# GeWu-Lab/Crab

Hardware: AMD Instinct MI355X
Metric: clips/sec prefill+decode (AVQA 10s clip, 8 frames, 256 out tok) (higher is better)
Workload: dtype bf16

## Files before the change

crab_amd/csrc/skinny.hip:

```cpp
#include "common.h"
#include "crab_internal.h"
#include "fp8_common.h"
#include "gemm_epilogue.h"
#include <stdlib.h>

namespace {

struct SkinnyP {
    const bf16_t* A; const bf16_t* B; void* C; const bf16_t* bias; const bf16_t* R;
    const bf16_t* A2; const bf16_t* B2;
    long lda, ldb, ldc, ldr, lda2, ldb2;
    int M, N, K, K2, act, c_fp32;
    float res_scale;
    const bf16_t* Bx; long ldbx; float* Tx;
    const float* rope_tab; bf16_t* rope_kc; bf16_t* rope_vc; const int* rope_pos_dev;
    int rope_H, rope_Hk, rope_d, rope_Tmax, rope_pos0;
    const int* rope_row_off;
    const uint8_t* B8; long ldb8; const float* bscale;
};

constexpr int SK_WAVES = 8;
constexpr int SKX = 8;

template <int MT, int NT>
__global__ __launch_bounds__(SK_WAVES * 64) void gemm_skinny_kernel(SkinnyP p) {
    constexpr int U = (NT + MT) <= 3 ? 4 : ((NT + MT) <= 6 ? 2 : 1);
    __shared__ __attribute__((aligned(16))) float red[SK_WAVES][NT * MT][64][4];
    const int tid = threadIdx.x, lane = tid & 63, wave = tid >> 6;
    const int fr = lane & 15, fg = lane >> 4;
    const int n0 = blockIdx.x * 16 * NT;

    const int ks1 = (p.K + 31) >> 5;
    const int ks2 = p.A2 ? (p.K2 + 31) >> 5 : 0;
    const int ks = ks1 + ks2;
    const int s_begin = (int)((long)ks * wave / SK_WAVES), s_end = (int)((long)ks * (wave + 1) / SK_WAVES);
    const int nst = s_end - s_begin;
    const int rot = nst > 0 ? (int)(blockIdx.x % (unsigned)nst) : 0;

    f32x4_t acc[NT][MT];
#pragma unroll
    for (int j = 0; j < NT; ++j)
#pragma unroll
        for (int i = 0; i < MT; ++i) acc[j][i] = f32x4_t{0.f, 0.f, 0.f, 0.f};
    long woff[NT];
#pragma unroll
    for (int j = 0; j < NT; ++j) woff[j] = min(n0 + j * 16 + fr, p.N - 1);
    int mrow[MT];
#pragma unroll
    for (int i = 0; i < MT; ++i) mrow[i] = min(i * 16 + fr, p.M - 1);

    const u32x4 z4 = {0u, 0u, 0u, 0u};
    for (int s = 0; s < nst; s += U) {
        u32x4 wv[U][NT], xv[U][MT];
#pragma unroll
        for (int u = 0; u < U; ++u) {
            const bool live = s + u < nst;
            int q = s + u + rot;
            if (q >= nst) q -= nst;
            const int st = live ? s_begin + q : s_begin;
            const bool seg2 = st >= ks1;
            const bf16_t* Bp = seg2 ? p.B2 : p.B;
            const bf16_t* Ap = seg2 ? p.A2 : p.A;
            const long lb = seg2 ? p.ldb2 : p.ldb, la = seg2 ? p.lda2 : p.lda;
            const int Kseg = seg2 ? p.K2 : p.K;
            const int k = ((seg2 ? st - ks1 : st) << 5) + fg * 8;
            const bool ok = live && k < Kseg;
            const int kc = ok ? k : 0;
#pragma unroll
            for (int j = 0; j < NT; ++j) {
                u32x4 w = *reinterpret_cast<const u32x4*>(Bp + woff[j] * lb + kc);
                wv[u][j] = ok ? w : z4;
            }
#pragma unroll
            for (int i = 0; i < MT; ++i) xv[u][i] = *reinterpret_cast<const u32x4*>(Ap + (long)mrow[i] * la + kc);
        }
#pragma unroll
        for (int u = 0; u < U; ++u) {
#pragma unroll
            for (int j = 0; j < NT; ++j) {
                union { u32x4 r; bf16x8_t f; } wf;
                wf.r = wv[u][j];
#pragma unroll
                for (int i = 0; i < MT; ++i) {
                    union { u32x4 r; bf16x8_t f; } xf;
                    xf.r = xv[u][i];
                    acc[j][i] = __builtin_amdgcn_mfma_f32_16x16x32_bf16(wf.f, xf.f, acc[j][i], 0, 0, 0);
                }
            }
        }
    }
#pragma unroll
    for (int j = 0; j < NT; ++j)
#pragma unroll
        for (int i = 0; i < MT; ++i) *reinterpret_cast<f32x4_t*>(&red[wave][j * MT + i][lane][0]) = acc[j][i];
    __syncthreads();

    for (int idx = tid; idx < NT * MT * 64; idx += SK_WAVES * 64) {
        const int t = idx >> 6, l = idx & 63;
        const int j = t / MT, i = t % MT;
        const int m = i * 16 + (l & 15);
        const int n = n0 + j * 16 + (l >> 4) * 4;
        if (m >= p.M || n >= p.N) continue;
        f32x4_t v = *reinterpret_cast<const f32x4_t*>(&red[0][t][l][0]);
#pragma unroll
        for (int w = 1; w < SK_WAVES; ++w) v += *reinterpret_cast<const f32x4_t*>(&red[w][t][l][0]);
        if (p.act == ACT_SWIGLU_PAIR) gemm_epilogue_scalar_swiglu(v, m, n, p.bias, p.C, p.ldc, p.c_fp32);
        else gemm_epilogue_scalar4(v, m, n, p.N, p.bias, p.act, p.R, p.ldr, p.res_scale, p.C, p.ldc, p.c_fp32);
    }
}

__device__ __attribute__((aligned(16))) uint32_t g_zero_page_sk[64];

typedef __attribute__((address_space(3))) void* sk_lds_vptr;
typedef const __attribute__((address_space(1))) void* sk_gbl_vptr;

struct SkRole {
    bool extra;
    int xe, n0, Nw;
    bool rope, r_qk;
    int r_hh, r_j, r_base, r_half;
    long wrow[2];
    int chunk[2];
    int fofs0, fofs1;
    __device__ __forceinline__ int rope_dim(int cg) const { return r_qk ? (cg >> 1) * r_half + 8 * r_j + (cg & 1) * 4 : 16 * r_j + cg * 4; }
};

template <int CH>
__device__ __forceinline__ SkRole sk_role(const SkinnyP& p, int lane) {
    SkRole k;
    const int nbN = (p.N + 15) / 16;
    k.extra = (int)blockIdx.x >= nbN;
    k.xe = (int)blockIdx.x - nbN;
    k.Nw = k.extra ? 16 : p.N;
    k.n0 = k.extra ? 0 : (int)blockIdx.x * 16;
    k.rope = p.rope_tab != nullptr && !k.extra;
    const int r_bpd = k.rope ? p.rope_d >> 4 : 1;
    k.r_hh = (int)blockIdx.x / r_bpd; k.r_j = (int)blockIdx.x % r_bpd;
    k.r_qk = k.rope && k.r_hh < p.rope_H + p.rope_Hk;
    k.r_base = k.r_hh * p.rope_d; k.r_half = p.rope_d >> 1;
#pragma unroll
    for (int i = 0; i < 2; ++i) {
        const int row = i * 8 + (lane >> 3);
        k.chunk[i] = (lane & 7) ^ ((row >> 1) & 7);
        k.wrow[i] = min(k.n0 + row, k.Nw - 1);
        if (k.r_qk) k.wrow[i] = k.r_base + (row >> 3) * k.r_half + 8 * k.r_j + (row & 7);
    }
    const int fr = lane & 15, fg = lane >> 4;
    k.fofs0 = fr * 8 * CH + ((fg ^ ((fr >> 1) & 7)) * CH);
    k.fofs1 = k.fofs0 ^ (4 * CH);
    return k;
}

template <typename V4>
__device__ __forceinline__ void sk_rope_tail(const SkinnyP& p, const SkRole& k, int l, const V4& s) {
    const int m = l & 15, cg = l >> 4;
    const int d = p.rope_d, pos = p.rope_pos0 + (p.rope_pos_dev ? p.rope_pos_dev[0] : 0);
    const int dim = k.rope_dim(cg);
    const int col = k.r_base + dim;
    float x[4], px[4];
#pragma unroll
    for (int r = 0; r < 4; ++r) {
        x[r] = bf2f(f2bf(s[r] + (p.bias ? bf2f(p.bias[col + r]) : 0.f)));
        px[r] = __shfl_xor(x[r], 32, 64);
    }
    if (m >= p.M) return;
    bf16_t* crow = reinterpret_cast<bf16_t*>(p.C) + (long)m * p.ldc + col;
    const uint32_t raw0 = pack_bf2(x[0], x[1]), raw1 = pack_bf2(x[2], x[3]);
    if (!k.r_qk) {
        const int hk = k.r_hh - p.rope_H - p.rope_Hk;
        *reinterpret_cast<u32x2*>(crow) = u32x2{raw0, raw1};
        *reinterpret_cast<u32x2*>(p.rope_vc + (((long)m * p.rope_Hk + hk) * p.rope_Tmax + pos) * d + dim) = u32x2{raw0, raw1};
        return;
    }
    const int idim = 8 * k.r_j + (cg & 1) * 4;
    const int rp = pos - (p.rope_row_off ? p.rope_row_off[m] : 0);
    const float* cs = p.rope_tab + ((long)rp * k.r_half + idim) * 2;
    float o[4];
#pragma unroll
    for (int r = 0; r < 4; ++r) {
        const float c = cs[2 * r], sn = cs[2 * r + 1];
        o[r] = cg < 2 ? rope_lo(x[r], px[r], c, sn) : rope_hi(px[r], x[r], c, sn);
    }
    const u32x2 ow = {pack_bf2(o[0], o[1]), pack_bf2(o[2], o[3])};
    if (k.r_hh < p.rope_H) {
        *reinterpret_cast<u32x2*>(crow) = ow;
    } else {
        const int hk = k.r_hh - p.rope_H;
        *reinterpret_cast<u32x2*>(crow) = u32x2{raw0, raw1};
        *reinterpret_cast<u32x2*>(p.rope_kc + (((long)m * p.rope_Hk + hk) * p.rope_Tmax + pos) * d + dim) = ow;
    }
}

template <typename V4>
__device__ __forceinline__ void sk_store(const SkinnyP& p, float* part, const V4& v, int m, int n) {
    if (part) gemm_epilogue_scalar4(v, m, n, p.N, p.bias, p.act, p.R, p.ldr, p.res_scale, part, p.N, CF_C32 | (p.c_fp32 & CF_R32));
    else if (p.act == ACT_SWIGLU_PAIR) gemm_epilogue_scalar_swiglu(v, m, n, p.bias, p.C, p.ldc, p.c_fp32);
    else gemm_epilogue_scalar4(v, m, n, p.N, p.bias, p.act, p.R, p.ldr, p.res_scale, p.C, p.ldc, p.c_fp32);
}

template <int NS>
__global__ __launch_bounds__(SK_WAVES * 64) void gemm_skinny_dma_kernel(SkinnyP p, float* __restrict__ part) {
    constexpr int SLOT = 16 * 64;
    __shared__ __attribute__((aligned(16))) bf16_t ring[SK_WAVES][NS][SLOT];
    __shared__ __attribute__((aligned(16))) float red[SK_WAVES][64][4];
    const int tid = threadIdx.x, lane = tid & 63;
    const int wave = __builtin_amdgcn_readfirstlane(tid >> 6);
    const int fr = lane & 15, fg = lane >> 4;
    const SkRole k = sk_role<8>(p, lane);
    const bf16_t* Bw = k.extra ? p.Bx : p.B;
    const long ldbw = k.extra ? p.ldbx : p.ldb;

    const int nk1 = (p.K + 63) >> 6;
    const int nk2 = (p.A2 && !k.extra) ? (p.K2 + 63) >> 6 : 0;
    const int kx0 = k.extra ? (int)((long)nk1 * k.xe / SKX) : 0;
    const int ks = k.extra ? (int)((long)nk1 * (k.xe + 1) / SKX) - kx0 : nk1 + nk2;
    const int s_begin = kx0 + (int)((long)ks * wave / SK_WAVES), s_end = kx0 + (int)((long)ks * (wave + 1) / SK_WAVES);
    const int nst = s_end - s_begin;

    const bf16_t* zero = reinterpret_cast<const bf16_t*>(g_zero_page_sk);
    long off1[2], off2[2];
    int kc[2];
#pragma unroll
    for (int i = 0; i < 2; ++i) {
        kc[i] = k.chunk[i] * 8;
        off1[i] = k.wrow[i] * ldbw + k.chunk[i] * 8;
        off2[i] = k.wrow[i] * p.ldb2 + k.chunk[i] * 8;
    }
    const long xrow1 = (long)min(fr, p.M - 1) * p.lda, xrow2 = (long)min(fr, p.M - 1) * p.lda2;
    bf16_t* myring = &ring[wave][0][0];

    u32x4 xv[NS][2];
#define SKD_STAGE(ST_, U_)                                                                                \
    {                                                                                                     \
        const int st_ = (ST_);                                                                            \
        const bool s2_ = st_ >= nk1;                                                                      \
        const int k0_ = (s2_ ? st_ - nk1 : st_) << 6;                                                     \
        const int Ks_ = s2_ ? p.K2 : p.K;                                                                 \
        _Pragma("unroll") for (int i = 0; i < 2; ++i) {                                                   \
            const bf16_t* src_ = (s2_ ? p.B2 + off2[i] : Bw + off1[i]) + k0_;                             \
            src_ = (k0_ + kc[i] < Ks_) ? src_ : zero;                                                     \
            __builtin_amdgcn_global_load_lds((sk_gbl_vptr)src_, (sk_lds_vptr)(myring + (U_) * SLOT + i * 512), 16, 0, 2);   \
        }                                                                                                 \
        _Pragma("unroll") for (int h = 0; h < 2; ++h) {                                                   \
            const int k_ = k0_ + h * 32 + fg * 8;                                                         \
            const int kk_ = k_ < Ks_ ? k_ : 0;                 \
            xv[U_][h] = *reinterpret_cast<const u32x4*>((s2_ ? p.A2 + xrow2 : p.A + xrow1) + kk_);        \
        }                                                                                                 \
    }

    f32x4_t acc = {0.f, 0.f, 0.f, 0.f};
#pragma unroll
    for (int u = 0; u < NS; ++u)
        if (u < nst) SKD_STAGE(s_begin + u, u)
    for (int s = 0; s < nst; s += NS) {
#pragma unroll
        for (int u = 0; u < NS; ++u) {
            if (s + u < nst) {
                if (s + u + NS - 1 < nst) asm volatile("s_waitcnt vmcnt(%0)" ::"n"((NS - 1) * 4) : "memory");
                else asm volatile("s_waitcnt vmcnt(0)" ::: "memory");
                union { u32x4 r; bf16x8_t f; } w0, w1, x0, x1;
                w0.r = *reinterpret_cast<const u32x4*>(myring + u * SLOT + k.fofs0);
                w1.r = *reinterpret_cast<const u32x4*>(myring + u * SLOT + k.fofs1);
                x0.r = xv[u][0]; x1.r = xv[u][1];
                acc = __builtin_amdgcn_mfma_f32_16x16x32_bf16(w0.f, x0.f, acc, 0, 0, 0);
                acc = __builtin_amdgcn_mfma_f32_16x16x32_bf16(w1.f, x1.f, acc, 0, 0, 0);
                asm volatile("" ::: "memory");
                if (s + u + NS < nst) SKD_STAGE(s_begin + s + u + NS, u)
            }
        }
    }
#undef SKD_STAGE
    *reinterpret_cast<f32x4_t*>(&red[wave][lane][0]) = acc;
    __syncthreads();
    if (tid >= 64) return;
    const int l = tid;
    const int m = l & 15, n = k.n0 + (l >> 4) * 4;
    if (!k.rope && (m >= p.M || n >= k.Nw)) return;
    f32x4_t v = *reinterpret_cast<const f32x4_t*>(&red[0][l][0]);
#pragma unroll
    for (int w = 1; w < SK_WAVES; ++w) v += *reinterpret_cast<const f32x4_t*>(&red[w][l][0]);
    if (k.rope) { sk_rope_tail(p, k, l, v); return; }
    if (k.extra) {
        *reinterpret_cast<f32x4_t*>(p.Tx + ((long)k.xe * 16 + m) * 16 + n) = v;
        return;
    }
    sk_store(p, part, v, m, n);
}

template <int NS>
__global__ __launch_bounds__(SK_WAVES * 64) void gemm_skinny_dma_w8_kernel(SkinnyP p, float* __restrict__ part) {
    constexpr int SLOTB = 16 * 128;
    __shared__ __attribute__((aligned(16))) uint8_t ring[SK_WAVES][NS][SLOTB];
    static_assert(NS * SLOTB >= 2 * 64 * 16, "the ring of a wave holds its two partial tiles");
    const int tid = threadIdx.x, lane = tid & 63;
    const int wave = __builtin_amdgcn_readfirstlane(tid >> 6);
    const int fr = lane & 15, fg = lane >> 4;
    const SkRole k = sk_role<16>(p, lane);

    const int nk64 = (p.K + 63) >> 6;
    const int nk8 = k.extra ? 0 : (p.K + 127) >> 7;
    const int nk2 = (p.A2 && !k.extra) ? (p.K2 + 63) >> 6 : 0;
    const int kx0 = k.extra ? (int)((long)nk64 * k.xe / SKX) : 0;
    const int ks = k.extra ? (int)((long)nk64 * (k.xe + 1) / SKX) - kx0 : nk8 + nk2;
    const int s_begin = kx0 + (int)((long)ks * wave / SK_WAVES), s_end = kx0 + (int)((long)ks * (wave + 1) / SK_WAVES);
    const int nst = s_end - s_begin;

    const uint8_t* zero = reinterpret_cast<const uint8_t*>(g_zero_page_sk);
    long off8[2], offb[2], off2[2];
    int kc[2];
#pragma unroll
    for (int i = 0; i < 2; ++i) {
        kc[i] = k.chunk[i];
        off8[i] = k.wrow[i] * p.ldb8 + k.chunk[i] * 16;
        offb[i] = (long)(k.extra ? i * 8 + (lane >> 3) : 0) * p.ldbx + k.chunk[i] * 8;
        off2[i] = k.wrow[i] * p.ldb2 + k.chunk[i] * 8;
    }
    const long xrow1 = (long)min(fr, p.M - 1) * p.lda, xrow2 = (long)min(fr, p.M - 1) * p.lda2;
    uint8_t* myring = &ring[wave][0][0];
    const int fofs0 = k.fofs0, fofs1 = k.fofs1;
    const int n8 = min(max(min(s_end, nk8) - s_begin, 0), nst);
    const int nb = nst - n8, sb_begin = s_begin + n8 - nk8;
    f32x4_t acc8 = {0.f, 0.f, 0.f, 0.f}, accb = {0.f, 0.f, 0.f, 0.f};
    {
        u32x4 xv[NS][4];
#define SK8_STAGE(ST_, U_)                                                                                \
        {                                                                                                 \
            const int k0_ = (ST_) << 7;                                                                   \
            _Pragma("unroll") for (int i = 0; i < 2; ++i) {                                               \
                const uint8_t* src_ = p.B8 + off8[i] + k0_;                                               \
                src_ = (k0_ + kc[i] * 16 < p.K) ? src_ : zero;                                            \
                __builtin_amdgcn_global_load_lds((sk_gbl_vptr)src_, (sk_lds_vptr)(myring + (U_) * SLOTB + i * 1024), 16, 0, 2);   \
            }                                                                                             \
            _Pragma("unroll") for (int h = 0; h < 4; ++h) {                                               \
                const int k_ = k0_ + (h >> 1) * 64 + fg * 16 + (h & 1) * 8;                               \
                const int kk_ = k_ < p.K ? k_ : 0;             \
                xv[U_][h] = *reinterpret_cast<const u32x4*>(p.A + xrow1 + kk_);                           \
            }                                                                                             \
        }
#pragma unroll
        for (int u = 0; u < NS; ++u)
            if (u < n8) SK8_STAGE(s_begin + u, u)
        for (int s = 0; s < n8; s += NS) {
#pragma unroll
            for (int u = 0; u < NS; ++u) {
                if (s + u < n8) {
                    if (s + u + NS - 1 < n8) asm volatile("s_waitcnt vmcnt(%0)" ::"n"((NS - 1) * 6) : "memory");
                    else asm volatile("s_waitcnt vmcnt(0)" ::: "memory");
                    u32x4 w0 = *reinterpret_cast<const u32x4*>(myring + u * SLOTB + fofs0);
                    u32x4 w1 = *reinterpret_cast<const u32x4*>(myring + u * SLOTB + fofs1);
                    const int kb = ((s_begin + s + u) << 7) + fg * 16 + 8;
                    const bool z0 = kb >= p.K, z1 = kb + 64 >= p.K;
                    w0[2] = z0 ? 0u : w0[2]; w0[3] = z0 ? 0u : w0[3];
                    w1[2] = z1 ? 0u : w1[2]; w1[3] = z1 ? 0u : w1[3];
                    union { u32x4 r; bf16x8_t f; } a0, a1, a2, a3, x0, x1, x2, x3;
                    a0.r = fp8x8_to_bf16x8(w0[0], w0[1]); a1.r = fp8x8_to_bf16x8(w0[2], w0[3]);
                    a2.r = fp8x8_to_bf16x8(w1[0], w1[1]); a3.r = fp8x8_to_bf16x8(w1[2], w1[3]);
                    x0.r = xv[u][0]; x1.r = xv[u][1]; x2.r = xv[u][2]; x3.r = xv[u][3];
                    acc8 = __builtin_amdgcn_mfma_f32_16x16x32_bf16(a0.f, x0.f, acc8, 0, 0, 0);
                    acc8 = __builtin_amdgcn_mfma_f32_16x16x32_bf16(a1.f, x1.f, acc8, 0, 0, 0);
                    acc8 = __builtin_amdgcn_mfma_f32_16x16x32_bf16(a2.f, x2.f, acc8, 0, 0, 0);
                    acc8 = __builtin_amdgcn_mfma_f32_16x16x32_bf16(a3.f, x3.f, acc8, 0, 0, 0);
                    asm volatile("" ::: "memory");
                    if (s + u + NS < n8) SK8_STAGE(s_begin + s + u + NS, u)
                }
            }
        }
#undef SK8_STAGE
    }
    if (nb > 0) {
        const bool s2 = !k.extra;
        const int Ks = s2 ? p.K2 : p.K;
        const bf16_t* zb = reinterpret_cast<const bf16_t*>(zero);
        const bf16_t* wb0 = s2 ? p.B2 + off2[0] : p.Bx + offb[0];
        const bf16_t* wb1 = s2 ? p.B2 + off2[1] : p.Bx + offb[1];
        const bf16_t* xb = s2 ? p.A2 + xrow2 : p.A + xrow1;
        u32x4 xw[NS][2];
#define SKB_STAGE(ST_, U_)                                                                                \
        {                                                                                                 \
            const int k0_ = (ST_) << 6;                                                                   \
            const bf16_t* s0_ = (k0_ + kc[0] * 8 < Ks) ? wb0 + k0_ : zb;                                  \
            const bf16_t* s1_ = (k0_ + kc[1] * 8 < Ks) ? wb1 + k0_ : zb;                                  \
            __builtin_amdgcn_global_load_lds((sk_gbl_vptr)s0_, (sk_lds_vptr)(myring + (U_) * SLOTB), 16, 0, 2);          \
            __builtin_amdgcn_global_load_lds((sk_gbl_vptr)s1_, (sk_lds_vptr)(myring + (U_) * SLOTB + 1024), 16, 0, 2);   \
            _Pragma("unroll") for (int h = 0; h < 2; ++h) {                                               \
                const int k_ = k0_ + h * 32 + fg * 8;                                                     \
                const int kk_ = k_ < Ks ? k_ : 0;                                                         \
                xw[U_][h] = *reinterpret_cast<const u32x4*>(xb + kk_);                                    \
            }                                                                                             \
        }
#pragma unroll
        for (int u = 0; u < NS; ++u)
            if (u < nb) SKB_STAGE(sb_begin + u, u)
        for (int s = 0; s < nb; s += NS) {
#pragma unroll
            for (int u = 0; u < NS; ++u) {
                if (s + u < nb) {
                    if (s + u + NS - 1 < nb) asm volatile("s_waitcnt vmcnt(%0)" ::"n"((NS - 1) * 4) : "memory");
                    else asm volatile("s_waitcnt vmcnt(0)" ::: "memory");
                    union { u32x4 r; bf16x8_t f; } b0, b1, x0, x1;
                    b0.r = *reinterpret_cast<const u32x4*>(myring + u * SLOTB + fofs0);
                    b1.r = *reinterpret_cast<const u32x4*>(myring + u * SLOTB + fofs1);
                    x0.r = xw[u][0]; x1.r = xw[u][1];
                    accb = __builtin_amdgcn_mfma_f32_16x16x32_bf16(b0.f, x0.f, accb, 0, 0, 0);
                    accb = __builtin_amdgcn_mfma_f32_16x16x32_bf16(b1.f, x1.f, accb, 0, 0, 0);
                    asm volatile("" ::: "memory");
                    if (s + u + NS < nb) SKB_STAGE(sb_begin + s + u + NS, u)
                }
            }
        }
#undef SKB_STAGE
    }
    float* myred = reinterpret_cast<float*>(myring);
    *reinterpret_cast<f32x4_t*>(myred + lane * 4) = acc8;
    *reinterpret_cast<f32x4_t*>(myred + 256 + lane * 4) = accb;
    __syncthreads();
    if (tid >= 64) return;
    const int l = tid;
    const int m = l & 15, n = k.n0 + (l >> 4) * 4;
    f32x4_t v8 = *reinterpret_cast<const f32x4_t*>(reinterpret_cast<const float*>(&ring[0][0][0]) + l * 4);
    f32x4_t vb = *reinterpret_cast<const f32x4_t*>(reinterpret_cast<const float*>(&ring[0][0][0]) + 256 + l * 4);
#pragma unroll
    for (int w = 1; w < SK_WAVES; ++w) {
        v8 += *reinterpret_cast<const f32x4_t*>(reinterpret_cast<const float*>(&ring[w][0][0]) + l * 4);
        vb += *reinterpret_cast<const f32x4_t*>(reinterpret_cast<const float*>(&ring[w][0][0]) + 256 + l * 4);
    }
    if (k.rope) {
        const int col = k.r_base + k.rope_dim(l >> 4);
        float t[4];
#pragma unroll
        for (int r = 0; r < 4; ++r) t[r] = __fmaf_rn(p.bscale[col + r], v8[r], vb[r]);
        sk_rope_tail(p, k, l, t);
        return;
    }
    if (m >= p.M || n >= k.Nw) return;
    if (k.extra) {
        *reinterpret_cast<f32x4_t*>(p.Tx + ((long)k.xe * 16 + m) * 16 + n) = vb;
        return;
    }
    float v[4];
#pragma unroll
    for (int r = 0; r < 4; ++r) v[r] = n + r < p.N ? __fmaf_rn(p.bscale[n + r], v8[r], vb[r]) : 0.f;
    sk_store(p, part, v, m, n);
}

template <int NT, int MT>
__global__ __launch_bounds__(256) void lora_t_partial_kernel(const bf16_t* __restrict__ X, long ldx, const bf16_t* __restrict__ RA, long ldra,
                                                             float* __restrict__ part, int M, int K, int kslice) {
    const int lane = threadIdx.x & 63, wave = threadIdx.x >> 6;
    const int fr = lane & 15, fg = lane >> 4;
    const int sl = blockIdx.x;
    const int m0 = (blockIdx.y * 4 + wave) * 16 * MT;
    if (m0 >= M) return;
    int mrow[MT];
#pragma unroll
    for (int i = 0; i < MT; ++i) mrow[i] = min(m0 + i * 16 + fr, M - 1);
    const int k_begin = sl * kslice, k_end = min(K, k_begin + kslice);
    f32x4_t acc[NT][MT];
#pragma unroll
    for (int j = 0; j < NT; ++j)
#pragma unroll
        for (int i = 0; i < MT; ++i) acc[j][i] = f32x4_t{0.f, 0.f, 0.f, 0.f};
    const u32x4 z4 = {0u, 0u, 0u, 0u};
    union Frag { u32x4 r; bf16x8_t f; };
    Frag xf[3][MT][2], wf[3][NT][2];
#define RT_LOAD(B_, K0_)                                                                                   \
    {                                                                                                      \
        _Pragma("unroll") for (int h = 0; h < 2; ++h) {                                                    \
            const int k_ = (K0_) + fg * 16 + h * 8;                                                        \
            _Pragma("unroll") for (int i = 0; i < MT; ++i)                                                 \
                xf[B_][i][h].r = *reinterpret_cast<const u32x4*>(X + (long)mrow[i] * ldx + k_);            \
            _Pragma("unroll") for (int j = 0; j < NT; ++j)                                                 \
                wf[B_][j][h].r = *reinterpret_cast<const u32x4*>(RA + (long)(j * 16 + fr) * ldra + k_);    \
        }                                                                                                  \
    }
#define RT_MMA(B_)                                                                                         \
    _Pragma("unroll") for (int h = 0; h < 2; ++h)                                                          \
        _Pragma("unroll") for (int j = 0; j < NT; ++j)                                                     \
            _Pragma("unroll") for (int i = 0; i < MT; ++i)                                                 \
                acc[j][i] = __builtin_amdgcn_mfma_f32_16x16x32_bf16(wf[B_][j][h].f, xf[B_][i][h].f, acc[j][i], 0, 0, 0);
    const int k_full = k_begin + ((k_end - k_begin) & ~63);
    int k0 = k_begin;
    if (k0 + 5 * 64 <= k_full) {
        RT_LOAD(0, k0);
        RT_LOAD(1, k0 + 64);
        for (; k0 + 5 * 64 <= k_full; k0 += 192) {
            RT_LOAD(2, k0 + 128);
            RT_MMA(0);
            RT_LOAD(0, k0 + 192);
            RT_MMA(1);
            RT_LOAD(1, k0 + 256);
            RT_MMA(2);
        }
        RT_MMA(0);
        RT_MMA(1);
        k0 += 128;
    }
    for (; k0 < k_full; k0 += 64) {
        RT_LOAD(0, k0);
        RT_MMA(0);
    }
    if (k_full < k_end) {
#pragma unroll
        for (int h = 0; h < 2; ++h) {
            const int k_ = k_full + fg * 16 + h * 8;
            const bool ok_ = k_ < k_end;
            const int kc_ = ok_ ? k_ : 0;
#pragma unroll
            for (int i = 0; i < MT; ++i) {
                xf[0][i][h].r = *reinterpret_cast<const u32x4*>(X + (long)mrow[i] * ldx + kc_);
                if (!ok_) xf[0][i][h].r = z4;
            }
#pragma unroll
            for (int j = 0; j < NT; ++j) wf[0][j][h].r = *reinterpret_cast<const u32x4*>(RA + (long)(j * 16 + fr) * ldra + kc_);
        }
        RT_MMA(0);
    }
#undef RT_LOAD
#undef RT_MMA
#pragma unroll
    for (int i = 0; i < MT; ++i) {
        const int m = m0 + i * 16 + fr;
        if (m < M) {
            float* o = part + ((long)sl * M + m) * (NT * 16);
#pragma unroll
            for (int j = 0; j < NT; ++j) *reinterpret_cast<f32x4_t*>(o + j * 16 + fg * 4) = acc[j][i];
        }
    }
}

__global__ __launch_bounds__(256) void lora_mix_reduce_kernel(const float* __restrict__ part, int nslices, int tcols, bf16_t* __restrict__ U,
                                                              long ldu, int M, int nproj, int nl, int r, int ucols, float scaling) {
    __shared__ float T[4][64];
    const int m0 = blockIdx.x * 4;
    const int tid = threadIdx.x;
    {
        const int row = tid >> 6, c = tid & 63;
        const int m = m0 + row;
        if (m < M && c < tcols) {
            float acc = 0.f;
            const float* q = part + (long)m * tcols + c;
            const long st = (long)M * tcols;
            int s = 0;
            for (; s + 8 <= nslices; s += 8) {
                float v[8];
#pragma unroll
                for (int i = 0; i < 8; ++i) v[i] = q[(s + i) * st];
#pragma unroll
                for (int i = 0; i < 8; ++i) acc += v[i];
            }
            for (; s < nslices; ++s) acc += q[s * st];
            T[row][c] = acc;
        }
    }
    __syncthreads();
    const int per_row = nproj + 1;
    if (tid >= 4 * per_row) return;
    const int row = tid / per_row, pj = tid % per_row;
    const int m = m0 + row;
    if (m >= M) return;
    bf16_t* u = U + (long)m * ldu;
    const int used = nproj * nl * r;
    if (pj == nproj) {
        for (int c = used; c < ucols; ++c) u[c] = 0;
        return;
    }
    const float* t = &T[row][pj * (nl + r)];
    float e[8], mx = -INFINITY;
    for (int i = 0; i < nl; ++i) mx = fmaxf(mx, t[i]);
    float sum = 0.f;
    for (int i = 0; i < nl; ++i) { e[i] = expf(t[i] - mx); sum += e[i]; }
    const float inv = 1.0f / sum;
    for (int i = 0; i < nl; ++i)
        for (int j = 0; j < r; ++j) u[pj * nl * r + i * r + j] = f2bf(scaling * e[i] * inv * t[nl + j]);
}


template <int MAXQ>
__global__ __launch_bounds__(256) void lora_route_row_kernel(const bf16_t* __restrict__ X, long ldx, const bf16_t* __restrict__ RA, long ldra, int K,
                                                             bf16_t* __restrict__ U, long ldu, int nproj, int nl, int r, int ucols, float scaling) {
    __shared__ float tp[48][257];
    __shared__ float tq[48][4];
    __shared__ float T[48];
    const int m = blockIdx.x, tid = threadIdx.x;
    float xv[MAXQ][8];
#pragma unroll
    for (int q = 0; q < MAXQ; ++q) {
        const int n = (tid + q * 256) * 8;
        u32x4 w = {0u, 0u, 0u, 0u};
        if (n < K) w = *reinterpret_cast<const u32x4*>(X + (long)m * ldx + n);
#pragma unroll
        for (int e = 0; e < 4; ++e) { xv[q][2 * e] = lo_bf(w[e]); xv[q][2 * e + 1] = hi_bf(w[e]); }
    }
    const int rows = nproj * (nl + r);
#define ROUTE_TRIPS(RPT_, NTRIPS_)                                                                        \
    for (int tr = 0; tr < (NTRIPS_); ++tr) {                                                              \
        const int c0 = tr * (RPT_);                                                                       \
        float p[RPT_];                                                                                    \
        _Pragma("unroll") for (int cc = 0; cc < (RPT_); ++cc) p[cc] = 0.f;                                \
        _Pragma("unroll") for (int q = 0; q < MAXQ; ++q) {                                                \
            const int n = (tid + q * 256) * 8;                                                            \
            if (n < K) {                                                                                  \
                u32x4 w[RPT_];                                                                            \
                _Pragma("unroll") for (int cc = 0; cc < (RPT_); ++cc)                                     \
                    w[cc] = c0 + cc < rows ? *reinterpret_cast<const u32x4*>(RA + (long)(c0 + cc) * ldra + n) : u32x4{0u, 0u, 0u, 0u};   \
                _Pragma("unroll") for (int cc = 0; cc < (RPT_); ++cc) {                                   \
                    float a = 0.f;                                                                        \
                    _Pragma("unroll") for (int e = 0; e < 4; ++e)                                         \
                        a += xv[q][2 * e] * lo_bf(w[cc][e]) + xv[q][2 * e + 1] * hi_bf(w[cc][e]);         \
                    p[cc] += a;                                                                           \
                }                                                                                         \
            }                                                                                             \
        }                                                                                                 \
        _Pragma("unroll") for (int cc = 0; cc < (RPT_); ++cc)                                             \
            if (c0 + cc < rows) tp[c0 + cc][tid] = p[cc];                                                 \
    }
    if (nl + r == 11) { ROUTE_TRIPS(11, nproj) }
    else { ROUTE_TRIPS(8, (rows + 7) / 8) }
#undef ROUTE_TRIPS
    __syncthreads();
    if (tid < rows * 4) {
        const int c = tid >> 2, qt = tid & 3;
        float a = 0.f;
        for (int i = qt * 64; i < qt * 64 + 64; ++i) a += tp[c][i];
        tq[c][qt] = a;
    }
    __syncthreads();
    if (tid < rows) T[tid] = (tq[tid][0] + tq[tid][1]) + (tq[tid][2] + tq[tid][3]);
    __syncthreads();
    if (tid > nproj) return;
    bf16_t* u = U + (long)m * ldu;
    const int used = nproj * nl * r;
    if (tid == nproj) {
        for (int c = used; c < ucols; ++c) u[c] = 0;
        return;
    }
    const float* t = &T[tid * (nl + r)];
    float e[8], mx = -INFINITY;
    for (int i = 0; i < nl; ++i) mx = fmaxf(mx, t[i]);
    float sum = 0.f;
    for (int i = 0; i < nl; ++i) { e[i] = expf(t[i] - mx); sum += e[i]; }
    const float inv = 1.0f / sum;
    for (int i = 0; i < nl; ++i)
        for (int j = 0; j < r; ++j) u[tid * nl * r + i * r + j] = f2bf(scaling * e[i] * inv * t[nl + j]);
}

template <int MAXQ>
__global__ __launch_bounds__(256) void lora_route_row2_kernel(const bf16_t* __restrict__ X, long ldx, const bf16_t* __restrict__ RA, long ldra, int M, int K,
                                                              bf16_t* __restrict__ U, long ldu, int nproj, int nl, int r, int ucols, float scaling) {
    constexpr int RMAX = 11;
    __shared__ float tp[2][RMAX][257];
    __shared__ float tq[2][RMAX][4];
    __shared__ float T[2][48];
    const int tid = threadIdx.x;
    const int m0 = blockIdx.x * 2;
    float xv[2][MAXQ][8];
#pragma unroll
    for (int rr = 0; rr < 2; ++rr) {
        const int m = min(m0 + rr, M - 1);
#pragma unroll
        for (int q = 0; q < MAXQ; ++q) {
            const int n = (tid + q * 256) * 8;
            u32x4 w = {0u, 0u, 0u, 0u};
            if (n < K) w = *reinterpret_cast<const u32x4*>(X + (long)m * ldx + n);
#pragma unroll
            for (int e = 0; e < 4; ++e) { xv[rr][q][2 * e] = lo_bf(w[e]); xv[rr][q][2 * e + 1] = hi_bf(w[e]); }
        }
    }
    const int rows = nproj * (nl + r);
#define ROUTE2_TRIPS(RPT_, NTRIPS_)                                                                       \
    for (int tr = 0; tr < (NTRIPS_); ++tr) {                                                              \
        const int c0 = tr * (RPT_);                                                                       \
        float p[2][RPT_];                                                                                 \
        _Pragma("unroll") for (int cc = 0; cc < (RPT_); ++cc) { p[0][cc] = 0.f; p[1][cc] = 0.f; }         \
        _Pragma("unroll") for (int q = 0; q < MAXQ; ++q) {                                                \
            const int n = (tid + q * 256) * 8;                                                            \
            if (n < K) {                                                                                  \
                u32x4 w[RPT_];                                                                            \
                _Pragma("unroll") for (int cc = 0; cc < (RPT_); ++cc)                                     \
                    w[cc] = c0 + cc < rows ? *reinterpret_cast<const u32x4*>(RA + (long)(c0 + cc) * ldra + n) : u32x4{0u, 0u, 0u, 0u};   \
                _Pragma("unroll") for (int rr = 0; rr < 2; ++rr)                                          \
                _Pragma("unroll") for (int cc = 0; cc < (RPT_); ++cc) {                                   \
                    float a = 0.f;                                                                        \
                    _Pragma("unroll") for (int e = 0; e < 4; ++e)                                         \
                        a += xv[rr][q][2 * e] * lo_bf(w[cc][e]) + xv[rr][q][2 * e + 1] * hi_bf(w[cc][e]); \
                    p[rr][cc] += a;                                                                       \
                }                                                                                         \
            }                                                                                             \
        }                                                                                                 \
        _Pragma("unroll") for (int rr = 0; rr < 2; ++rr)                                                  \
        _Pragma("unroll") for (int cc = 0; cc < (RPT_); ++cc) tp[rr][cc][tid] = p[rr][cc];                \
        __syncthreads();                                                                                  \
        if (tid < 2 * (RPT_) * 4) {                                                                       \
            const int rr = tid / ((RPT_) * 4), c = (tid % ((RPT_) * 4)) >> 2, qt = tid & 3;               \
            float a = 0.f;                                                                                \
            for (int i = qt * 64; i < qt * 64 + 64; ++i) a += tp[rr][c][i];                               \
            tq[rr][c][qt] = a;                                                                            \
        }                                                                                                 \
        __syncthreads();                                                                                  \
        if (tid < 2 * (RPT_)) {                                                                           \
            const int rr = tid / (RPT_), c = tid % (RPT_);                                                \
            if (c0 + c < rows) T[rr][c0 + c] = (tq[rr][c][0] + tq[rr][c][1]) + (tq[rr][c][2] + tq[rr][c][3]);   \
        }                                                                                                 \
    }
    static_assert(RMAX * 4 * 2 <= 256, "quarter sums: one thread per (row, router row, quarter)");
    if (nl + r == 11) { ROUTE2_TRIPS(11, nproj) }
    else { ROUTE2_TRIPS(8, (rows + 7) / 8) }
#undef ROUTE2_TRIPS
    __syncthreads();
    const int rr = tid >> 7, lt = tid & 127;
    const int m = m0 + rr;
    if (m >= M || lt > nproj) return;
    bf16_t* u = U + (long)m * ldu;
    const int used = nproj * nl * r;
    if (lt == nproj) {
        for (int c = used; c < ucols; ++c) u[c] = 0;
        return;
    }
    const float* t = &T[rr][lt * (nl + r)];
    float e[8], mx = -INFINITY;
    for (int i = 0; i < nl; ++i) mx = fmaxf(mx, t[i]);
    float sum = 0.f;
    for (int i = 0; i < nl; ++i) { e[i] = expf(t[i] - mx); sum += e[i]; }
    const float inv = 1.0f / sum;
    for (int i = 0; i < nl; ++i)
        for (int j = 0; j < r; ++j) u[lt * nl * r + i * r + j] = f2bf(scaling * e[i] * inv * t[nl + j]);
}

}

float* crab_rowfin_T(const crab_gemm_desc* d);

bool crab_skinny_fuses_rope(const crab_gemm_desc* d) {
    static const int on = []() { const char* e = getenv("CRAB_SKINNY_ROPE"); return !(e && e[0] == '0'); }();
    return on && d->rope_tab && d->M <= 16 && d->tune == 0 && !d->c_fp32 && (d->rope_d & 15) == 0 && d->rope_d >= 16 && (d->ldc & 3) == 0 &&
           (d->ldb & 7) == 0 && (!d->A2 || (d->ldb2 & 7) == 0) && d->N == (d->rope_H + 2 * d->rope_Hk) * d->rope_d &&
           (((uintptr_t)d->C | (uintptr_t)d->rope_k_cache | (uintptr_t)d->rope_v_cache) & 7) == 0;
}

int crab_gemm_skinny_launch(crab_ctx* ctx, hipStream_t s, const crab_gemm_desc* d) {
    SkinnyP p;
    p.A = (const bf16_t*)d->A; p.B = (const bf16_t*)d->B; p.C = d->C; p.bias = (const bf16_t*)d->bias; p.R = (const bf16_t*)d->R;
    p.A2 = (const bf16_t*)d->A2; p.B2 = (const bf16_t*)d->B2;
    p.lda = d->lda; p.ldb = d->ldb; p.ldc = d->ldc; p.ldr = d->ldr; p.lda2 = d->lda2; p.ldb2 = d->ldb2;
    p.M = d->M; p.N = d->N; p.K = d->K; p.K2 = d->A2 ? d->K2 : 0; p.act = d->act; p.c_fp32 = crab_cflags(d); p.res_scale = d->res_scale;
    p.Bx = nullptr; p.ldbx = 0; p.Tx = nullptr;
    p.rope_tab = nullptr; p.rope_kc = p.rope_vc = nullptr; p.rope_pos_dev = nullptr; p.rope_H = p.rope_Hk = p.rope_d = p.rope_Tmax = p.rope_pos0 = 0;
    p.rope_row_off = nullptr;
    p.B8 = nullptr; p.ldb8 = 0; p.bscale = nullptr;
    if (crab_skinny_fuses_rope(d)) {
        p.rope_tab = d->rope_tab; p.rope_kc = (bf16_t*)d->rope_k_cache; p.rope_vc = (bf16_t*)d->rope_v_cache; p.rope_pos_dev = d->rope_pos_dev;
        p.rope_H = d->rope_H; p.rope_Hk = d->rope_Hk; p.rope_d = d->rope_d; p.rope_Tmax = d->rope_Tmax; p.rope_pos0 = d->rope_pos0;
        p.rope_row_off = d->rope_row_off;
    }
    if (d->M <= 16 && (d->tune == 0 || d->tune == 9) && (d->ldb & 7) == 0 && (!d->A2 || (d->ldb2 & 7) == 0)) {
        float* part = d->tune == 9 ? (float*)d->workspace : nullptr;
        int extra_blocks = 0;
        if (d->tune == 9 && d->lora_RA) {
            p.Bx = (const bf16_t*)d->lora_RA; p.ldbx = d->lora_ldra; p.Tx = crab_rowfin_T(d);
            extra_blocks = SKX;
        }
        if (d->B8) {
            p.B8 = (const uint8_t*)d->B8; p.ldb8 = d->ldb8; p.bscale = d->b_scale;
            hipLaunchKernelGGL((gemm_skinny_dma_w8_kernel<4>), dim3((d->N + 15) / 16 + extra_blocks), dim3(SK_WAVES * 64), 0, s, p, part);
            return crab_check_launch(ctx, "gemm_skinny_dma_w8_kernel");
        }
        hipLaunchKernelGGL((gemm_skinny_dma_kernel<4>), dim3((d->N + 15) / 16 + extra_blocks), dim3(SK_WAVES * 64), 0, s, p, part);
        return crab_check_launch(ctx, "gemm_skinny_dma_kernel");
    }
    if (d->B8) return crab_fail(ctx, CRAB_E_UNSUPPORTED, "gemm: FP8 weights (B8) need the M <= 16 LDS-DMA kernel (tune 0 / 9, ldb and ldb2 multiples of 8)");
    int mt = d->M <= 16 ? 1 : (d->M <= 32 ? 2 : (d->M <= 64 ? 4 : 8));
    int nt = d->tune > 0 ? d->tune : 0;
    if (nt == 0) {
        nt = 1;
        if (mt >= 2 && d->N >= 8192) nt = 2;
        if (mt >= 4 && d->N >= 16384) nt = 4;
    }
    if (nt != 1 && nt != 2 && nt != 4) nt = 1;
    if (mt == 8 && nt == 4) nt = 2;
    dim3 grid((d->N + 16 * nt - 1) / (16 * nt)), block(SK_WAVES * 64);
#define SK_LAUNCH(MT_, NT_) hipLaunchKernelGGL((gemm_skinny_kernel<MT_, NT_>), grid, block, 0, s, p)
#define SK_NT(MT_) do { if (nt == 1) SK_LAUNCH(MT_, 1); else if (nt == 2) SK_LAUNCH(MT_, 2); else SK_LAUNCH(MT_, 4); } while (0)
    if (mt == 1) SK_NT(1);
    else if (mt == 2) SK_NT(2);
    else if (mt == 4) SK_NT(4);
    else { if (nt == 1) SK_LAUNCH(8, 1); else SK_LAUNCH(8, 2); }
#undef SK_NT
#undef SK_LAUNCH
    return crab_check_launch(ctx, "gemm_skinny_kernel");
}

static int route_slices(int M, int K) {
    int mblocks = (M + 63) / 64;
    int nslices = (1024 + mblocks - 1) / (mblocks > 0 ? mblocks : 1);
    int maxs = (K + 127) / 128;
    if (nslices > maxs) nslices = maxs;
    if (nslices < 1) nslices = 1;
    if (nslices > 16) nslices = 16;
    return nslices;
}

static void route_cfg(int M, int K, int* MT, int* nslices) {
    *MT = M >= 4096 ? 4 : 1;
    *nslices = route_slices(*MT == 4 ? (M + 3) / 4 : M, K);
}

extern "C" int64_t crab_hyperlora_route_workspace(int M, int K, int tcols) {
    if (M <= 0 || K <= 0 || tcols <= 0) return 0;
    const int64_t maxs = (K + 127) / 128 < 16 ? (K + 127) / 128 : 16;
    int64_t rows = maxs * (int64_t)M;
    if (rows > 262144 + (int64_t)M) rows = 262144 + (int64_t)M;
    return rows * tcols * (int64_t)sizeof(float);
}

extern "C" int crab_hyperlora_route(crab_ctx* ctx, void* stream, const void* X, int64_t ldx, const void* RA, int64_t ldra, int M, int K,
                                    int nproj, int nl, int r, void* U, int64_t ldu, int ucols, float scaling, void* workspace,
                                    int64_t workspace_bytes) {
    if (!ctx) return CRAB_E_INVALID;
    if (!X || !RA || !U || !workspace || M <= 0 || K <= 0 || (K & 7) || (ldx & 7) || (ldra & 7))
        return crab_fail(ctx, CRAB_E_INVALID, "hyperlora_route: bad argument");
    if (nproj < 1 || nl < 1 || nl > 8 || r < 1 || ucols < nproj * nl * r) return crab_fail(ctx, CRAB_E_INVALID, "hyperlora_route: nproj, r >= 1, 1 <= nl <= 8, ucols >= nproj nl r");
    const int tcols = ((nproj * (nl + r) + 15) / 16) * 16;
    if (crab_hyperlora_route_workspace(M, K, tcols) > workspace_bytes) return crab_fail(ctx, CRAB_E_WORKSPACE, "hyperlora_route: workspace too small");
    if (nl + r > 16 || nproj > 3 || tcols > 64) {
        crab_gemm_desc g;
        memset(&g, 0, sizeof(g));
        g.A = X; g.lda = ldx; g.B = RA; g.ldb = ldra; g.C = workspace; g.ldc = tcols; g.M = M; g.N = tcols; g.K = K;
        g.c_fp32 = 1; g.res_scale = 1.0f; g.batch = 1; g.nb0 = 1;
        int rc = crab_gemm_bf16(ctx, stream, &g);
        return rc ? rc : crab_hyperlora_mix(ctx, stream, workspace, tcols, 1, U, ldu, M, nproj, nl, r, ucols, scaling);
    }
    if (M > 64 && M <= CRAB_DECODE_MAX_ROWS && K <= 6 * 2048 && nl <= 8 && ((uintptr_t)X & 15) == 0 && ((uintptr_t)RA & 15) == 0) {
        hipStream_t s0 = (hipStream_t)stream;
#define RR_LAUNCH(Q_) hipLaunchKernelGGL((lora_route_row_kernel<Q_>), dim3(M), dim3(256), 0, s0, (const bf16_t*)X, (long)ldx, (const bf16_t*)RA, (long)ldra, K, \
                                         (bf16_t*)U, (long)ldu, nproj, nl, r, ucols, scaling)
        const char* e1 = getenv("CRAB_ROUTE_ROWS");
        if (M > 256 && K > 4 * 2048 && !(e1 && e1[0] == '1' && e1[1] == 0)) {
            hipLaunchKernelGGL((lora_route_row2_kernel<6>), dim3((M + 1) / 2), dim3(256), 0, s0, (const bf16_t*)X, (long)ldx, (const bf16_t*)RA, (long)ldra, M, K,
                               (bf16_t*)U, (long)ldu, nproj, nl, r, ucols, scaling);
            return crab_check_launch(ctx, "lora_route_row2_kernel");
        }
        if (K <= 2 * 2048) RR_LAUNCH(2); else if (K <= 4 * 2048) RR_LAUNCH(4); else RR_LAUNCH(6);
#undef RR_LAUNCH
        return crab_check_launch(ctx, "lora_route_row_kernel");
    }
    int MT, nslices;
    route_cfg(M, K, &MT, &nslices);
    int mblocks = (M + 64 * MT - 1) / (64 * MT);
    hipStream_t s = (hipStream_t)stream;
    int kslice = (((K + nslices - 1) / nslices) + 63) / 64 * 64;
    nslices = (K + kslice - 1) / kslice;
    dim3 grid(nslices, mblocks), block(256);
    float* part = (float*)workspace;
    const int NT = tcols / 16;
#define RT_LAUNCH(NT_, MT_) hipLaunchKernelGGL((lora_t_partial_kernel<NT_, MT_>), grid, block, 0, s, (const bf16_t*)X, (long)ldx, (const bf16_t*)RA, \
                                               (long)ldra, part, M, K, kslice)
    if (MT == 4) { if (NT == 1) RT_LAUNCH(1, 4); else if (NT == 2) RT_LAUNCH(2, 4); else RT_LAUNCH(3, 4); }
    else { if (NT == 1) RT_LAUNCH(1, 1); else if (NT == 2) RT_LAUNCH(2, 1); else RT_LAUNCH(3, 1); }
#undef RT_LAUNCH
    int rc = crab_check_launch(ctx, "lora_t_partial_kernel");
    if (rc) return rc;
    if (tcols > 64) return crab_fail(ctx, CRAB_E_UNSUPPORTED, "hyperlora_route: tcols <= 64");
    unsigned blocks = (unsigned)((M + 3) / 4);
    hipLaunchKernelGGL(lora_mix_reduce_kernel, dim3(blocks), dim3(256), 0, s, part, nslices, tcols, (bf16_t*)U, (long)ldu, M, nproj, nl, r, ucols, scaling);
    return crab_check_launch(ctx, "lora_mix_reduce_kernel");
}
```

Baseline: 31.01.

## Software-pipeline LoRA router loads and parallelize router reductions across waves

Rewrites the two LoRA routing kernels around a shared helper. The helper double-buffers router-weight loads so the next chunk, or the next trip's first chunk, is fetched while the current one is multiplied. It also pads the shared partial-sum buffer to avoid bank conflicts, replaces the serial quarter sums with vectorized loads plus cross-lane shuffles, and spreads the softmax mixing and zero fill across a wave's lanes instead of single threads. The cost is more register pressure from the double buffers and scheduling barriers, and clamped loads now fetch redundant rows and columns.

```diff
diff --git a/crab_amd/csrc/route_core.h b/crab_amd/csrc/route_core.h
--- /dev/null
+++ b/crab_amd/csrc/route_core.h
@@ -0,0 +1,99 @@
+#pragma once
+#include "common.h"
+
+constexpr int ROUTE_TP_LD = 272;
+__device__ __forceinline__ int route_tp_col(int t) { return t + ((t >> 6) << 2); }
+
+template <int RPT>
+__device__ __forceinline__ void route_ld(u32x4 (&w)[11], const bf16_t* __restrict__ RA, long ldra, int c0, int rows, int n, int N) {
+    static_assert(RPT <= 11, "the chunk buffer");
+    const bf16_t* col = RA + min(n, N - 8);
+#pragma unroll
+    for (int cc = 0; cc < RPT; ++cc) w[cc] = *reinterpret_cast<const u32x4*>(col + (long)min(c0 + cc, rows - 1) * ldra);
+}
+
+template <int RPT, int MAXQ, int NR, typename F>
+__device__ __forceinline__ void route_trips(const float (&xv)[NR][MAXQ][8], const bf16_t* __restrict__ RA, long ldra, int rows, int N, int tid,
+                                            int ntrips, u32x4 (&w0)[11], F&& done) {
+    static_assert(MAXQ % 2 == 0, "the buffer of the next trip's first chunk");
+    const int nqb = min(MAXQ, (N + 2047) / 2048);
+    const int nqe = (nqb + 1) & ~1;
+    for (int tr = 0; tr < ntrips; ++tr) {
+        int c0 = tr * RPT;
+        asm volatile("" : "+s"(c0));
+        u32x4 w1[11];
+        float p[NR][RPT];
+#pragma unroll
+        for (int rr = 0; rr < NR; ++rr)
+#pragma unroll
+            for (int cc = 0; cc < RPT; ++cc) p[rr][cc] = 0.f;
+#pragma unroll
+        for (int q = 0; q < MAXQ; ++q) {
+            if (q < nqe) {
+                const int n = (tid + q * 256) * 8;
+                u32x4 (&w)[11] = (q & 1) ? w1 : w0;
+                if (q + 1 < nqb) route_ld<RPT>((q & 1) ? w0 : w1, RA, ldra, c0, rows, n + 2048, N);
+                else if ((q & 1) && q + 1 == nqe && tr + 1 < ntrips) route_ld<RPT>(w0, RA, ldra, c0 + RPT, rows, tid * 8, N);
+                __builtin_amdgcn_sched_barrier(0);
+                if (n < N) {
+#pragma unroll
+                    for (int cc = 0; cc < RPT; ++cc) {
+#pragma unroll
+                        for (int rr = 0; rr < NR; ++rr) {
+                            float a = 0.f;
+#pragma unroll
+                            for (int e = 0; e < 4; ++e) a += xv[rr][q][2 * e] * lo_bf(w[cc][e]) + xv[rr][q][2 * e + 1] * hi_bf(w[cc][e]);
+                            p[rr][cc] += a;
+                        }
+                        __builtin_amdgcn_sched_barrier(0);
+                    }
+                }
+            }
+        }
+        done(tr, p);
+    }
+}
+
+__device__ __forceinline__ float route_quarter(const float* row, int qt) {
+    const f32x4_t* src = reinterpret_cast<const f32x4_t*>(row + qt * 68);
+    f32x4_t v[16];
+#pragma unroll
+    for (int k = 0; k < 16; ++k) v[k] = src[k];
+    float a = 0.f;
+#pragma unroll
+    for (int k = 0; k < 16; ++k) { a += v[k][0]; a += v[k][1]; a += v[k][2]; a += v[k][3]; }
+    return a;
+}
+
+__device__ __forceinline__ float route_quad(float a) {
+    a = a + row_xor1(a);
+    return a + row_xor2(a);
+}
+
+__device__ __forceinline__ void route_mix(const float* t, bf16_t* __restrict__ u, int nl, int r, float scaling, int lane) {
+    float mx = -INFINITY;
+    for (int i = 0; i < nl; ++i) mx = fmaxf(mx, t[i]);
+    float sum = 0.f;
+    for (int i = 0; i < nl; ++i) sum += expf(t[i] - mx);
+    const float inv = 1.0f / sum;
+    for (int k = lane; k < nl * r; k += 64) {
+        const int i = k / r, j = k - i * r;
+        u[k] = f2bf(scaling * expf(t[i] - mx) * inv * t[nl + j]);
+    }
+}
+
+__device__ __forceinline__ void route_tail(const float (*tp)[ROUTE_TP_LD], float* T, int tid, int nproj, int nl, int r, bf16_t* __restrict__ u,
+                                           float scaling) {
+    const int lane = tid & 63, wave = tid >> 6, g = nl + r, rows = nproj * g;
+    const bool local = g <= 16 && nproj <= 4;
+    const int rw = local ? g : 16;
+    const int c = wave * rw + (lane >> 2);
+    const bool on = (lane >> 2) < rw && c < rows;
+    float a = 0.f;
+    if (on) a = route_quarter(tp[c], lane & 3);
+    a = route_quad(a);
+    if (on && (lane & 3) == 0) T[c] = a;
+    if (local) __builtin_amdgcn_wave_barrier();
+    else __syncthreads();
+    for (int p = wave; p < nproj; p += 4) route_mix(&T[p * g], u + p * nl * r, nl, r, scaling, lane);
+}
diff --git a/crab_amd/csrc/skinny.hip b/crab_amd/csrc/skinny.hip
--- a/crab_amd/csrc/skinny.hip
+++ b/crab_amd/csrc/skinny.hip
@@ -2,6 +2,7 @@
 #include "crab_internal.h"
 #include "fp8_common.h"
 #include "gemm_epilogue.h"
+#include "route_core.h"
 #include <stdlib.h>
 
 namespace {
@@ -578,152 +579,96 @@
 template <int MAXQ>
 __global__ __launch_bounds__(256) void lora_route_row_kernel(const bf16_t* __restrict__ X, long ldx, const bf16_t* __restrict__ RA, long ldra, int K,
                                                              bf16_t* __restrict__ U, long ldu, int nproj, int nl, int r, int ucols, float scaling) {
-    __shared__ float tp[48][257];
-    __shared__ float tq[48][4];
+    __shared__ __align__(16) float tp[48][ROUTE_TP_LD];
     __shared__ float T[48];
     const int m = blockIdx.x, tid = threadIdx.x;
-    float xv[MAXQ][8];
+    const int g = nl + r, rows = nproj * g;
+    u32x4 xw[MAXQ], w0[11];
 #pragma unroll
     for (int q = 0; q < MAXQ; ++q) {
         const int n = (tid + q * 256) * 8;
-        u32x4 w = {0u, 0u, 0u, 0u};
-        if (n < K) w = *reinterpret_cast<const u32x4*>(X + (long)m * ldx + n);
-#pragma unroll
-        for (int e = 0; e < 4; ++e) { xv[q][2 * e] = lo_bf(w[e]); xv[q][2 * e + 1] = hi_bf(w[e]); }
-    }
-    const int rows = nproj * (nl + r);
-#define ROUTE_TRIPS(RPT_, NTRIPS_)                                                                        \
-    for (int tr = 0; tr < (NTRIPS_); ++tr) {                                                              \
-        const int c0 = tr * (RPT_);                                                                       \
-        float p[RPT_];                                                                                    \
-        _Pragma("unroll") for (int cc = 0; cc < (RPT_); ++cc) p[cc] = 0.f;                                \
-        _Pragma("unroll") for (int q = 0; q < MAXQ; ++q) {                                                \
-            const int n = (tid + q * 256) * 8;                                                            \
-            if (n < K) {                                                                                  \
-                u32x4 w[RPT_];                                                                            \
-                _Pragma("unroll") for (int cc = 0; cc < (RPT_); ++cc)                                     \
-                    w[cc] = c0 + cc < rows ? *reinterpret_cast<const u32x4*>(RA + (long)(c0 + cc) * ldra + n) : u32x4{0u, 0u, 0u, 0u};   \
-                _Pragma("unroll") for (int cc = 0; cc < (RPT_); ++cc) {                                   \
-                    float a = 0.f;                                                                        \
-                    _Pragma("unroll") for (int e = 0; e < 4; ++e)                                         \
-                        a += xv[q][2 * e] * lo_bf(w[cc][e]) + xv[q][2 * e + 1] * hi_bf(w[cc][e]);         \
-                    p[cc] += a;                                                                           \
-                }                                                                                         \
-            }                                                                                             \
-        }                                                                                                 \
-        _Pragma("unroll") for (int cc = 0; cc < (RPT_); ++cc)                                             \
-            if (c0 + cc < rows) tp[c0 + cc][tid] = p[cc];                                                 \
-    }
-    if (nl + r == 11) { ROUTE_TRIPS(11, nproj) }
-    else { ROUTE_TRIPS(8, (rows + 7) / 8) }
-#undef ROUTE_TRIPS
+        xw[q] = u32x4{0u, 0u, 0u, 0u};
+        if (n < K) xw[q] = *reinterpret_cast<const u32x4*>(X + (long)m * ldx + n);
+    }
+    if (g == 11) route_ld<11>(w0, RA, ldra, 0, rows, tid * 8, K);
+    else route_ld<8>(w0, RA, ldra, 0, rows, tid * 8, K);
+    float xv[1][MAXQ][8];
+#pragma unroll
+    for (int q = 0; q < MAXQ; ++q)
+#pragma unroll
+        for (int e = 0; e < 4; ++e) { xv[0][q][2 * e] = lo_bf(xw[q][e]); xv[0][q][2 * e + 1] = hi_bf(xw[q][e]); }
+    bf16_t* u = U + (long)m * ldu;
+    for (int c = nproj * nl * r + tid; c < ucols; c += 256) u[c] = 0;
+    if (g == 11)
+        route_trips<11, MAXQ, 1>(xv, RA, ldra, rows, K, tid, nproj, w0, [&](int tr, const float (&p)[1][11]) {
+#pragma unroll
+            for (int cc = 0; cc < 11; ++cc) tp[tr * 11 + cc][route_tp_col(tid)] = p[0][cc];
+        });
+    else
+        route_trips<8, MAXQ, 1>(xv, RA, ldra, rows, K, tid, (rows + 7) / 8, w0, [&](int tr, const float (&p)[1][8]) {
+#pragma unroll
+            for (int cc = 0; cc < 8; ++cc)
+                if (tr * 8 + cc < rows) tp[tr * 8 + cc][route_tp_col(tid)] = p[0][cc];
+        });
     __syncthreads();
-    if (tid < rows * 4) {
-        const int c = tid >> 2, qt = tid & 3;
-        float a = 0.f;
-        for (int i = qt * 64; i < qt * 64 + 64; ++i) a += tp[c][i];
-        tq[c][qt] = a;
-    }
-    __syncthreads();
-    if (tid < rows) T[tid] = (tq[tid][0] + tq[tid][1]) + (tq[tid][2] + tq[tid][3]);
-    __syncthreads();
-    if (tid > nproj) return;
-    bf16_t* u = U + (long)m * ldu;
-    const int used = nproj * nl * r;
-    if (tid == nproj) {
-        for (int c = used; c < ucols; ++c) u[c] = 0;
-        return;
-    }
-    const float* t = &T[tid * (nl + r)];
-    float e[8], mx = -INFINITY;
-    for (int i = 0; i < nl; ++i) mx = fmaxf(mx, t[i]);
-    float sum = 0.f;
-    for (int i = 0; i < nl; ++i) { e[i] = expf(t[i] - mx); sum += e[i]; }
-    const float inv = 1.0f / sum;
-    for (int i = 0; i < nl; ++i)
-        for (int j = 0; j < r; ++j) u[tid * nl * r + i * r + j] = f2bf(scaling * e[i] * inv * t[nl + j]);
+    route_tail(tp, T, tid, nproj, nl, r, u, scaling);
 }
 
 template <int MAXQ>
 __global__ __launch_bounds__(256) void lora_route_row2_kernel(const bf16_t* __restrict__ X, long ldx, const bf16_t* __restrict__ RA, long ldra, int M, int K,
                                                               bf16_t* __restrict__ U, long ldu, int nproj, int nl, int r, int ucols, float scaling) {
     constexpr int RMAX = 11;
-    __shared__ float tp[2][RMAX][257];
-    __shared__ float tq[2][RMAX][4];
+    __shared__ __align__(16) float tp[2][2][RMAX][ROUTE_TP_LD];
     __shared__ float T[2][48];
-    const int tid = threadIdx.x;
+    const int tid = threadIdx.x, lane = tid & 63, wave = tid >> 6;
     const int m0 = blockIdx.x * 2;
-    float xv[2][MAXQ][8];
+    const int g = nl + r, rows = nproj * g;
+    u32x4 xw[2][MAXQ], w0[11];
 #pragma unroll
     for (int rr = 0; rr < 2; ++rr) {
         const int m = min(m0 + rr, M - 1);
 #pragma unroll
         for (int q = 0; q < MAXQ; ++q) {
             const int n = (tid + q * 256) * 8;
-            u32x4 w = {0u, 0u, 0u, 0u};
-            if (n < K) w = *reinterpret_cast<const u32x4*>(X + (long)m * ldx + n);
-#pragma unroll
-            for (int e = 0; e < 4; ++e) { xv[rr][q][2 * e] = lo_bf(w[e]); xv[rr][q][2 * e + 1] = hi_bf(w[e]); }
-        }
-    }
-    const int rows = nproj * (nl + r);
-#define ROUTE2_TRIPS(RPT_, NTRIPS_)                                                                       \
-    for (int tr = 0; tr < (NTRIPS_); ++tr) {                                                              \
-        const int c0 = tr * (RPT_);                                                                       \
-        float p[2][RPT_];                                                                                 \
-        _Pragma("unroll") for (int cc = 0; cc < (RPT_); ++cc) { p[0][cc] = 0.f; p[1][cc] = 0.f; }         \
-        _Pragma("unroll") for (int q = 0; q < MAXQ; ++q) {                                                \
-            const int n = (tid + q * 256) * 8;                                                            \
-            if (n < K) {                                                                                  \
-                u32x4 w[RPT_];                                                                            \
-                _Pragma("unroll") for (int cc = 0; cc < (RPT_); ++cc)                                     \
-                    w[cc] = c0 + cc < rows ? *reinterpret_cast<const u32x4*>(RA + (long)(c0 + cc) * ldra + n) : u32x4{0u, 0u, 0u, 0u};   \
-                _Pragma("unroll") for (int rr = 0; rr < 2; ++rr)                                          \
-                _Pragma("unroll") for (int cc = 0; cc < (RPT_); ++cc) {                                   \
-                    float a = 0.f;                                                                        \
-                    _Pragma("unroll") for (int e = 0; e < 4; ++e)                                         \
-                        a += xv[rr][q][2 * e] * lo_bf(w[cc][e]) + xv[rr][q][2 * e + 1] * hi_bf(w[cc][e]); \
-                    p[rr][cc] += a;                                                                       \
-                }                                                                                         \
-            }                                                                                             \
+            xw[rr][q] = u32x4{0u, 0u, 0u, 0u};
+            if (n < K) xw[rr][q] = *reinterpret_cast<const u32x4*>(X + (long)m * ldx + n);
+        }
+    }
+    if (g == 11) route_ld<11>(w0, RA, ldra, 0, rows, tid * 8, K);
+    else route_ld<8>(w0, RA, ldra, 0, rows, tid * 8, K);
+    float xv[2][MAXQ][8];
+#pragma unroll
+    for (int rr = 0; rr < 2; ++rr)
+#pragma unroll
+        for (int q = 0; q < MAXQ; ++q)
+#pragma unroll
+            for (int e = 0; e < 4; ++e) { xv[rr][q][2 * e] = lo_bf(xw[rr][q][e]); xv[rr][q][2 * e + 1] = hi_bf(xw[rr][q][e]); }
+    if (m0 + (tid >> 7) < M) {
+        bf16_t* uz = U + (long)(m0 + (tid >> 7)) * ldu;
+        for (int c = nproj * nl * r + (tid & 127); c < ucols; c += 128) uz[c] = 0;
+    }
+#define ROUTE2_DONE(RPT_)                                                                                 \
+    [&](int tr, const float (&p)[2][RPT_]) {                                                              \
+        float (*buf)[RMAX][ROUTE_TP_LD] = tp[tr & 1];                                                     \
+        _Pragma("unroll") for (int rr = 0; rr < 2; ++rr)                                                  \
+        _Pragma("unroll") for (int cc = 0; cc < (RPT_); ++cc) buf[rr][cc][route_tp_col(tid)] = p[rr][cc]; \
+        __syncthreads();                                                                                  \
+        if (wave < 2) {                                                                                   \
+            const int c = lane >> 2;                                                                      \
+            const bool on = c < (RPT_) && tr * (RPT_) + c < rows;                                         \
+            float a = 0.f;                                                                                \
+            if (on) a = route_quarter(buf[wave][c], lane & 3);                                            \
+            a = route_quad(a);                                                                            \
+            if (on && (lane & 3) == 0) T[wave][tr * (RPT_) + c] = a;                                      \
         }                                                                                                 \
-        _Pragma("unroll") for (int rr = 0; rr < 2; ++rr)                                                  \
-        _Pragma("unroll") for (int cc = 0; cc < (RPT_); ++cc) tp[rr][cc][tid] = p[rr][cc];                \
-        __syncthreads();                                                                                  \
-        if (tid < 2 * (RPT_) * 4) {                                                                       \
-            const int rr = tid / ((RPT_) * 4), c = (tid % ((RPT_) * 4)) >> 2, qt = tid & 3;               \
-            float a = 0.f;                                                                                \
-            for (int i = qt * 64; i < qt * 64 + 64; ++i) a += tp[rr][c][i];                               \
-            tq[rr][c][qt] = a;                                                                            \
-        }                                                                                                 \
-        __syncthreads();                                                                                  \
-        if (tid < 2 * (RPT_)) {                                                                           \
-            const int rr = tid / (RPT_), c = tid % (RPT_);                                                \
-            if (c0 + c < rows) T[rr][c0 + c] = (tq[rr][c][0] + tq[rr][c][1]) + (tq[rr][c][2] + tq[rr][c][3]);   \
-        }                                                                                                 \
-    }
-    static_assert(RMAX * 4 * 2 <= 256, "quarter sums: one thread per (row, router row, quarter)");
-    if (nl + r == 11) { ROUTE2_TRIPS(11, nproj) }
-    else { ROUTE2_TRIPS(8, (rows + 7) / 8) }
-#undef ROUTE2_TRIPS
-    __syncthreads();
-    const int rr = tid >> 7, lt = tid & 127;
-    const int m = m0 + rr;
-    if (m >= M || lt > nproj) return;
-    bf16_t* u = U + (long)m * ldu;
-    const int used = nproj * nl * r;
-    if (lt == nproj) {
-        for (int c = used; c < ucols; ++c) u[c] = 0;
-        return;
-    }
-    const float* t = &T[rr][lt * (nl + r)];
-    float e[8], mx = -INFINITY;
-    for (int i = 0; i < nl; ++i) mx = fmaxf(mx, t[i]);
-    float sum = 0.f;
-    for (int i = 0; i < nl; ++i) { e[i] = expf(t[i] - mx); sum += e[i]; }
-    const float inv = 1.0f / sum;
-    for (int i = 0; i < nl; ++i)
-        for (int j = 0; j < r; ++j) u[lt * nl * r + i * r + j] = f2bf(scaling * e[i] * inv * t[nl + j]);
+    }
+    if (g == 11) route_trips<11, MAXQ, 2>(xv, RA, ldra, rows, K, tid, nproj, w0, ROUTE2_DONE(11));
+    else route_trips<8, MAXQ, 2>(xv, RA, ldra, rows, K, tid, (rows + 7) / 8, w0, ROUTE2_DONE(8));
+#undef ROUTE2_DONE
+    const int m = m0 + wave;
+    if (wave >= 2 || m >= M) return;
+    __builtin_amdgcn_wave_barrier();
+    for (int pj = 0; pj < nproj; ++pj) route_mix(&T[wave][pj * g], U + (long)m * ldu + pj * nl * r, nl, r, scaling, lane);
 }
 
 }
```

After: 31.04 (median of 5 runs). About the same (+0.1%).
